# WHU-USI3DV/GAGS

Measured on AMD Instinct MI355X. Metric: feature-raster fwd+bwd views/s, higher is better.
Workload: dtype f32

## Files before the change

### gags_amd/csrc/rows_reduce.hip

```cpp
#include <hip/hip_fp16.h>
#include "launch.h"

namespace {

__global__ __launch_bounds__(256) void row_tail_kernel(int64_t cap, const int32_t *__restrict__ total, int n_gauss,
                                                       uint32_t *__restrict__ row_key, int32_t *__restrict__ row_idx)
{
    const int64_t i = (int64_t)blockIdx.x * 256 + threadIdx.x;
    if (i >= cap || i < (int64_t)total[0]) return;
    row_key[i] = (uint32_t)n_gauss;
    row_idx[i] = 0;
}

__global__ __launch_bounds__(256) void seg_offsets_kernel(int n, const uint32_t *__restrict__ sorted_keys, int n_keys,
                                                          int32_t *__restrict__ seg)
{
    const int i = blockIdx.x * 256 + threadIdx.x;
    if (i >= n) return;
    const int cur = min((int)sorted_keys[i], n_keys);
    if (i == 0) {
        for (int g = 0; g <= cur; ++g) seg[g] = 0;
    } else {
        const int prev = min((int)sorted_keys[i - 1], n_keys);
        for (int g = prev + 1; g <= cur; ++g) seg[g] = i;
    }
    if (i == n - 1)
        for (int g = cur + 1; g <= n_keys; ++g) seg[g] = n;
}

__global__ void seg_fill_kernel(int n_keys, int32_t *__restrict__ seg)
{
    const int g = blockIdx.x * 256 + threadIdx.x;
    if (g <= n_keys) seg[g] = 0;
}

constexpr int REDUCE_ITER = 8;
template <bool HALF, int VW>
__global__ __launch_bounds__(256) void reduce_rows_kernel(int n_gauss, int d, int ch_begin, int ch_count,
                                                          const int32_t *__restrict__ seg,
                                                          const int32_t *__restrict__ sorted_rows,
                                                          const float *__restrict__ prow, int prow_pitch,
                                                          void *__restrict__ v_colors_, int sparse,
                                                          const int32_t *__restrict__ wire_pos, float *__restrict__ wire,
                                                          const uint8_t *__restrict__ keep_prev, uint8_t *__restrict__ keep_cur,
                                                          int tail)
{
    const int lpg = ch_count / VW;
    const int gpb = 256 / lpg;
    const int gl = threadIdx.x / lpg;
    const int cl = ch_begin + (threadIdx.x % lpg) * VW;
    if (gl >= gpb) return;
    for (int it = 0; it < REDUCE_ITER; ++it) {
    const int g = (blockIdx.x * REDUCE_ITER + it) * gpb + gl;
    if (g >= n_gauss) return;
        const int b = seg[g], e = seg[g + 1];
        const bool has = b != e;
        bool write_grad = sparse ? has : true;
        const bool on_wire = wire && wire_pos[g] >= 0;
        if (keep_cur) {
            if (threadIdx.x % lpg == 0) keep_cur[g] = (has || on_wire) ? 1 : 0;
            write_grad = has || keep_prev[g] != 0;
        }
        if (!write_grad && !on_wire) continue;
        const bool skip_grad = !write_grad;
        if constexpr (VW == 1) {
            float acc = 0.f;
            for (int i = b; i < e; ++i) acc += prow[(size_t)sorted_rows[i] * prow_pitch + cl];
            if (!skip_grad) {
                if constexpr (HALF) reinterpret_cast<__half *>(v_colors_)[(size_t)g * d + cl] = __float2half_rn(acc);
                else reinterpret_cast<float *>(v_colors_)[(size_t)g * d + cl] = acc;
            }
            if (wire) {
                const int q = wire_pos[g];
                if (q >= 0) wire[(size_t)q * ch_count + (cl - ch_begin)] = acc;
            }
        } else {
            float4 acc = make_float4(0.f, 0.f, 0.f, 0.f);
            const int tl = threadIdx.x % lpg;
            const bool has_tail = tl < tail;
            const int ct = ch_begin + ch_count + (has_tail ? tl : 0);
            float acc_t = 0.f;
            for (int i = b; i < e; i += 8) {
                int r[8];
#pragma unroll
                for (int j = 0; j < 8; ++j) r[j] = sorted_rows[min(i + j, e - 1)];
                float4 v[8];
                float vt[8];
#pragma unroll
                for (int j = 0; j < 8; ++j) {
                    v[j] = *reinterpret_cast<const float4 *>(prow + (size_t)r[j] * prow_pitch + cl);
                    vt[j] = has_tail ? prow[(size_t)r[j] * prow_pitch + ct] : 0.f;
                }
#pragma unroll
                for (int j = 0; j < 8; ++j) {
                    if (i + j < e) {
                        acc.x += v[j].x; acc.y += v[j].y; acc.z += v[j].z; acc.w += v[j].w;
                        acc_t += vt[j];
                    }
                }
            }
            if (!skip_grad && has_tail) {
                if constexpr (HALF) reinterpret_cast<__half *>(v_colors_)[(size_t)g * d + ct] = __float2half_rn(acc_t);
                else reinterpret_cast<float *>(v_colors_)[(size_t)g * d + ct] = acc_t;
            }
            if (!skip_grad) {
                if constexpr (HALF) {
                    const __half2 lo = __floats2half2_rn(acc.x, acc.y), hi = __floats2half2_rn(acc.z, acc.w);
                    uint2 w;
                    w.x = *reinterpret_cast<const unsigned *>(&lo);
                    w.y = *reinterpret_cast<const unsigned *>(&hi);
                    *reinterpret_cast<uint2 *>(reinterpret_cast<__half *>(v_colors_) + (size_t)g * d + cl) = w;
                } else {
                    typedef float nt_f4 __attribute__((ext_vector_type(4)));
                    __builtin_nontemporal_store(nt_f4{acc.x, acc.y, acc.z, acc.w},
                                                reinterpret_cast<nt_f4 *>(reinterpret_cast<float *>(v_colors_) + (size_t)g * d + cl));
                }
            }
            if (wire) {
                const int q = wire_pos[g];
                if (q >= 0) *reinterpret_cast<float4 *>(wire + (size_t)q * ch_count + (cl - ch_begin)) = acc;
            }
        }
    }
}

}

int gags_rows_group_launch(int64_t rows, int n_gauss, const int32_t *rows_dev, uint32_t *key, int32_t *idx, uint32_t *key_s,
                           int32_t *idx_s, int32_t *seg, void *sort_scratch, int64_t sort_scratch_bytes, hipStream_t st)
{
    if (rows <= 0) {
        hipLaunchKernelGGL(seg_fill_kernel, dim3((n_gauss + 1 + 255) / 256), dim3(256), 0, st, n_gauss, seg);
        return GAGS_OK;
    }
    const dim3 grid((unsigned)((rows + 255) / 256));
    if (rows_dev) hipLaunchKernelGGL(row_tail_kernel, grid, dim3(256), 0, st, rows, rows_dev, n_gauss, key, idx);
    int nbits = 1;
    while ((1ll << nbits) <= n_gauss) ++nbits;
    const int rc = gags_sort_pairs_u32(rows, nbits, key, idx, key_s, idx_s, sort_scratch, sort_scratch_bytes, st);
    if (rc != GAGS_OK) return rc;
    hipLaunchKernelGGL(seg_offsets_kernel, grid, dim3(256), 0, st, (int)rows, key_s, n_gauss, seg);
    return GAGS_OK;
}

int gags_rows_reduce_launch(int n_gauss, int d, int ch_begin, int ch_count, const int32_t *seg, const int32_t *idx_s,
                            const float *prow, int pitch, void *out, bool out_f16, hipStream_t st, int sparse,
                            const int32_t *wire_pos, float *wire, const uint8_t *keep_prev, uint8_t *keep_cur)
{
    const int c4 = ch_count & ~3, c1 = ch_count & 3;
    if (wire && (c1 != 0 || !wire_pos)) return GAGS_EINVAL;
    const bool ride = c4 >= 16 && c1 > 0;
    auto reduce = [&](auto *k_f16, auto *k_f32, int vw, int c0, int cw, int tail) {
        const int gpb = 256 / (cw / vw);
        const dim3 grid((n_gauss + gpb * REDUCE_ITER - 1) / (gpb * REDUCE_ITER));
        hipLaunchKernelGGL(out_f16 ? k_f16 : k_f32, grid, dim3(256), 0, st, n_gauss, d, c0, cw, seg, idx_s, prow, pitch, out, sparse,
                           wire_pos, wire, keep_prev, keep_cur, tail);
    };
    if (c4 > 0) reduce((reduce_rows_kernel<true, 4>), (reduce_rows_kernel<false, 4>), 4, ch_begin, c4, ride ? c1 : 0);
    if (c1 > 0 && !ride) reduce((reduce_rows_kernel<true, 1>), (reduce_rows_kernel<false, 1>), 1, ch_begin + c4, c1, 0);
    return GAGS_OK;
}
```

Measured before the change: 132.5.

## Add run-based row reduction kernel sharing segment metadata across consecutive Gaussians

Adds a new reduction kernel where each lane group handles a run of eight consecutive Gaussians. Segment bounds, wire positions and keep flags are loaded once per lane and broadcast through readlane or shuffle. Sorted row indices are prefetched cooperatively and broadcast, and row loads are double-buffered in batches of four, so short segments no longer leave lanes idle. The launcher picks this kernel when lanes per Gaussian are 16, 32, 64 or 128, at the cost of more complex control flow and serial handling of segment boundaries.

Measured after the change: 130.7. -1.3%, worse.

```diff
diff --git a/gags_amd/csrc/rows_reduce.hip b/gags_amd/csrc/rows_reduce.hip
--- a/gags_amd/csrc/rows_reduce.hip
+++ b/gags_amd/csrc/rows_reduce.hip
@@ -124,6 +124,145 @@
     }
 }
 
+constexpr int REDUCE_RUN = 8;
+constexpr int REDUCE_BATCH = 4;
+
+template <int GL>
+__device__ __forceinline__ int run_bcast(int v, int lane)
+{
+    if constexpr (GL == 64) return __builtin_amdgcn_readlane(v, lane);
+    else return __shfl(v, lane, GL);
+}
+
+template <bool HALF, int GL>
+__global__ __launch_bounds__(256) void reduce_rows_run_kernel(int n_gauss, int d, int ch_begin, int ch_count,
+                                                              const int32_t *__restrict__ seg,
+                                                              const int32_t *__restrict__ sorted_rows,
+                                                              const float *__restrict__ prow, int prow_pitch,
+                                                              void *__restrict__ v_colors_, int sparse,
+                                                              const int32_t *__restrict__ wire_pos, float *__restrict__ wire,
+                                                              const uint8_t *__restrict__ keep_prev, uint8_t *__restrict__ keep_cur,
+                                                              int tail)
+{
+    static_assert(REDUCE_RUN < GL && GL % REDUCE_BATCH == 0, "lane k holds Gaussian k's metadata; a batch stays inside one round");
+    const int lpg = ch_count / 4;
+    const int gpb = 256 / lpg;
+    const int tl = threadIdx.x % lpg;
+    const int sl = threadIdx.x % GL;
+    const int cl = ch_begin + tl * 4;
+    int g0 = (blockIdx.x * gpb + threadIdx.x / lpg) * REDUCE_RUN;
+    if constexpr (GL == 64) g0 = __builtin_amdgcn_readfirstlane(g0);
+    if (g0 >= n_gauss) return;
+    const bool has_tail = tl < tail;
+    const int ct = ch_begin + ch_count + (has_tail ? tl : 0);
+
+    const int gk = g0 + sl;
+    const bool mine = sl < REDUCE_RUN && gk < n_gauss;
+    int sa = 0, sb = 0, wp = -1, kp = 0;
+    if (sl <= REDUCE_RUN) sa = seg[min(gk, n_gauss)];
+    if (mine) {
+        sb = seg[gk + 1];
+        if (wire) wp = wire_pos[gk];
+        if (keep_cur) kp = keep_prev[gk];
+    }
+    int fl = 0;
+    if (mine) {
+        const bool has = sa != sb, on_wire = wp >= 0;
+        bool write_grad = sparse ? has : true;
+        if (keep_cur) {
+            if (tl < GL) keep_cur[gk] = (has || on_wire) ? 1 : 0;
+            write_grad = has || kp != 0;
+        }
+        fl = (write_grad ? 1 : 0) | (on_wire ? 2 : 0);
+    }
+    const int s0 = run_bcast<GL>(sa, 0), sn = run_bcast<GL>(sa, REDUCE_RUN);
+
+    float4 acc = make_float4(0.f, 0.f, 0.f, 0.f);
+    float acc_t = 0.f;
+    int k = 0;
+    int end_k = run_bcast<GL>(sa, 1);
+    auto finish = [&](int kk) {
+        const int f = run_bcast<GL>(fl, kk);
+        if (f != 0) {
+            const int g = g0 + kk;
+            if (f & 1) {
+                if (has_tail) {
+                    if constexpr (HALF) reinterpret_cast<__half *>(v_colors_)[(size_t)g * d + ct] = __float2half_rn(acc_t);
+                    else reinterpret_cast<float *>(v_colors_)[(size_t)g * d + ct] = acc_t;
+                }
+                if constexpr (HALF) {
+                    const __half2 lo = __floats2half2_rn(acc.x, acc.y), hi = __floats2half2_rn(acc.z, acc.w);
+                    uint2 w;
+                    w.x = *reinterpret_cast<const unsigned *>(&lo);
+                    w.y = *reinterpret_cast<const unsigned *>(&hi);
+                    *reinterpret_cast<uint2 *>(reinterpret_cast<__half *>(v_colors_) + (size_t)g * d + cl) = w;
+                } else {
+                    typedef float nt_f4 __attribute__((ext_vector_type(4)));
+                    __builtin_nontemporal_store(nt_f4{acc.x, acc.y, acc.z, acc.w},
+                                                reinterpret_cast<nt_f4 *>(reinterpret_cast<float *>(v_colors_) + (size_t)g * d + cl));
+                }
+            }
+            if (f & 2) {
+                const int q = run_bcast<GL>(wp, kk);
+                *reinterpret_cast<float4 *>(wire + (size_t)q * ch_count + (cl - ch_begin)) = acc;
+            }
+        }
+        acc = make_float4(0.f, 0.f, 0.f, 0.f);
+        acc_t = 0.f;
+    };
+
+    if (s0 < sn) {
+        int base = s0, rv = sorted_rows[min(s0 + sl, sn - 1)], rvn = 0;
+        if (s0 + GL < sn) rvn = sorted_rows[min(s0 + GL + sl, sn - 1)];
+        auto request = [&](int p, float4 (&v)[REDUCE_BATCH], float (&vt)[REDUCE_BATCH]) {
+            if (p - base >= GL) {
+                base += GL;
+                rv = rvn;
+                if (base + GL < sn) rvn = sorted_rows[min(base + GL + sl, sn - 1)];
+            }
+#pragma unroll
+            for (int j = 0; j < REDUCE_BATCH; ++j) {
+                const int r = run_bcast<GL>(rv, min(p + j, sn - 1) - base);
+                v[j] = *reinterpret_cast<const float4 *>(prow + (size_t)r * prow_pitch + cl);
+                vt[j] = has_tail ? prow[(size_t)r * prow_pitch + ct] : 0.f;
+            }
+        };
+        auto add = [&](int p, const float4 (&v)[REDUCE_BATCH], const float (&vt)[REDUCE_BATCH]) {
+#pragma unroll
+            for (int j = 0; j < REDUCE_BATCH; ++j) {
+                if (p + j < sn) {
+                    while (p + j >= end_k) {
+                        finish(k);
+                        ++k;
+                        end_k = run_bcast<GL>(sa, k + 1);
+                    }
+                    acc.x += v[j].x; acc.y += v[j].y; acc.z += v[j].z; acc.w += v[j].w;
+                    acc_t += vt[j];
+                }
+            }
+        };
+        float4 va[REDUCE_BATCH], vb[REDUCE_BATCH];
+        float ta[REDUCE_BATCH], tb[REDUCE_BATCH];
+        int p = s0;
+        request(p, va, ta);
+        while (p + 2 * REDUCE_BATCH < sn) {
+            request(p + REDUCE_BATCH, vb, tb);
+            add(p, va, ta);
+            request(p + 2 * REDUCE_BATCH, va, ta);
+            add(p + REDUCE_BATCH, vb, tb);
+            p += 2 * REDUCE_BATCH;
+        }
+        if (p + REDUCE_BATCH < sn) {
+            request(p + REDUCE_BATCH, vb, tb);
+            add(p, va, ta);
+            add(p + REDUCE_BATCH, vb, tb);
+        } else {
+            add(p, va, ta);
+        }
+    }
+    for (; k < REDUCE_RUN; ++k) finish(k);
+}
+
 }
 
 int gags_rows_group_launch(int64_t rows, int n_gauss, const int32_t *rows_dev, uint32_t *key, int32_t *idx, uint32_t *key_s,
@@ -150,13 +289,17 @@
     const int c4 = ch_count & ~3, c1 = ch_count & 3;
     if (wire && (c1 != 0 || !wire_pos)) return GAGS_EINVAL;
     const bool ride = c4 >= 16 && c1 > 0;
-    auto reduce = [&](auto *k_f16, auto *k_f32, int vw, int c0, int cw, int tail) {
+    auto reduce = [&](auto *k_f16, auto *k_f32, int vw, int c0, int cw, int tail, int per) {
         const int gpb = 256 / (cw / vw);
-        const dim3 grid((n_gauss + gpb * REDUCE_ITER - 1) / (gpb * REDUCE_ITER));
+        const dim3 grid((n_gauss + gpb * per - 1) / (gpb * per));
         hipLaunchKernelGGL(out_f16 ? k_f16 : k_f32, grid, dim3(256), 0, st, n_gauss, d, c0, cw, seg, idx_s, prow, pitch, out, sparse,
                            wire_pos, wire, keep_prev, keep_cur, tail);
     };
-    if (c4 > 0) reduce((reduce_rows_kernel<true, 4>), (reduce_rows_kernel<false, 4>), 4, ch_begin, c4, ride ? c1 : 0);
-    if (c1 > 0 && !ride) reduce((reduce_rows_kernel<true, 1>), (reduce_rows_kernel<false, 1>), 1, ch_begin + c4, c1, 0);
+    const int lpg = c4 / 4;
+    if (lpg == 64 || lpg == 128) reduce((reduce_rows_run_kernel<true, 64>), (reduce_rows_run_kernel<false, 64>), 4, ch_begin, c4, ride ? c1 : 0, REDUCE_RUN);
+    else if (lpg == 32) reduce((reduce_rows_run_kernel<true, 32>), (reduce_rows_run_kernel<false, 32>), 4, ch_begin, c4, ride ? c1 : 0, REDUCE_RUN);
+    else if (lpg == 16) reduce((reduce_rows_run_kernel<true, 16>), (reduce_rows_run_kernel<false, 16>), 4, ch_begin, c4, ride ? c1 : 0, REDUCE_RUN);
+    else if (c4 > 0) reduce((reduce_rows_kernel<true, 4>), (reduce_rows_kernel<false, 4>), 4, ch_begin, c4, ride ? c1 : 0, REDUCE_ITER);
+    if (c1 > 0 && !ride) reduce((reduce_rows_kernel<true, 1>), (reduce_rows_kernel<false, 1>), 1, ch_begin + c4, c1, 0, REDUCE_ITER);
     return GAGS_OK;
 }
```
